# yanielc/medical-vision-textural-bias

Hardware: AMD Instinct MI355X
Metric: BraTS 4ch 240^3 vols/sec filtered+train-step @1/2/4/8 GPU; filter HBM GB/s (higher is better)
Workload: dtype f32

## Files before the change

medical-vision-textural-bias_amd/csrc/conv_gemm.hip:

```cpp
#include <hip/hip_runtime.h>

#include <cstdint>
#include <cstdlib>

#include "gemm_core.h"
#include "num_cu.h"
#include "texbias.h"

namespace {

using namespace tb::gemm;

struct CGArgs {
  const float* x;
  const float* A;
  const float* bias;
  const float* add;
  float* y;
  float* part;
  int64_t xsn, ysn, addsn;
  int64_t xbytes;
  int xsc, ysc;
  int Cin, M;
  int IDm, IH, IW;
  int OD, OH, OW;
  int YH, YW;
  int S, ymul;
  int P;
  int nsplit, kper, mtiles, ptiles, ncls;
  int kind;
  int64_t aoff[8];
  int Kc[8], Tc[8];
};

__host__ __device__ inline void tap_of(int kind, int cls, int j, int& dz, int& dy, int& dx, int& widx) {
  if (kind == 0) {
    dz = j / 9 - 1, dy = (j / 3) % 3 - 1, dx = j % 3 - 1, widx = j;
  } else if (kind == 1) {
    dz = dy = dx = 0, widx = 0;
  } else {
    const int pz = (cls >> 2) & 1, py = (cls >> 1) & 1, px = cls & 1;
    const int nx = 1 + px, ny = 1 + py;
    const int ix = j % nx, iy = (j / nx) % ny, iz = j / (nx * ny);
    dz = pz ? iz : 0, dy = py ? iy : 0, dx = px ? ix : 0;
    const int tz = pz ? (iz ? 0 : 2) : 1, ty = py ? (iy ? 0 : 2) : 1, tx = px ? (ix ? 0 : 2) : 1;
    widx = tz * 9 + ty * 3 + tx;
  }
}

template <int BM, int BP, int WGM>
__global__ __launch_bounds__(NTH) void k_conv_gemm(const CGArgs a) {
  using TileT = Tile<BM, BP, WGM>;
  constexpr int NPOS = BP / 64;
  constexpr int AQ = BM * KC / 4 / NTH;
  static_assert(NPOS >= 1 && AQ >= 1, "tile");
  extern __shared__ __attribute__((aligned(16))) float lds_dyn[];
  const int tid = (int)threadIdx.x, lane = tid & 63;
  const int w = __builtin_amdgcn_readfirstlane(tid >> 6);
  int b = xcd_remap((int)blockIdx.x, (int)gridDim.x);
  const int mt = b % a.mtiles;
  b /= a.mtiles;
  const int pt = b % a.ptiles;
  b /= a.ptiles;
  const int split = b % a.nsplit, cls = b / a.nsplit;
  const int T = a.Tc[cls], K = a.Kc[cls];
  const float* __restrict__ A = a.A + a.aoff[cls];
  const int Cin = a.Cin;
  const int k_beg = split * a.kper;
  const int k_end = min(K, k_beg + a.kper);
  const int m0 = mt * BM, p0 = pt * BP;
  const int IHW = a.IH * a.IW;

  int xo[NPOS];
  uint32_t vm[NPOS];
#pragma unroll
  for (int i = 0; i < NPOS; ++i) {
    const int p = p0 + lane + 64 * i;
    const bool ok = p < a.P;
    int t = ok ? p : 0;
    const int ox = t % a.OW;
    t /= a.OW;
    const int oy = t % a.OH;
    t /= a.OH;
    const int oz = t % a.OD, n = t / a.OD;
    const int bz = a.S * oz, by = a.S * oy, bx = a.S * ox;
    xo[i] = 4 * ((int)(n * a.xsn) + bz * IHW + by * a.IW + bx);
    uint32_t m = 0;
    for (int j = 0; j < T; ++j) {
      int dz, dy, dx, wi;
      tap_of(a.kind, cls, j, dz, dy, dx, wi);
      const int iz = bz + dz, iy = by + dy, ix = bx + dx;
      const bool v = ok && iz >= 0 && iz < a.IDm && iy >= 0 && iy < a.IH && ix >= 0 && ix < a.IW;
      m |= (v ? 1u : 0u) << j;
    }
    vm[i] = m;
  }
  const uint32_t xbytes = (uint32_t)__builtin_amdgcn_readfirstlane((int)a.xbytes);
  const __amdgpu_buffer_rsrc_t xr = __builtin_amdgcn_make_buffer_rsrc(const_cast<float*>(a.x), 0, (int)xbytes, 0x00020000);
  const int xsc4 = 4 * a.xsc;

  float rb[2][NPOS][8];
  f32x4 ra[2][AQ];
  auto gather = [&](auto SL, int k0) {
    constexpr int sl = decltype(SL)::value;
    const int k = k0 + 8 * w;
    const int t = k / Cin, c = k - t * Cin;
    const bool kin = k < k_end;
    int dz, dy, dx, wi;
    tap_of(a.kind, cls, kin ? t : 0, dz, dy, dx, wi);
    const int off = 4 * ((dz * a.IH + dy) * a.IW + dx);
    const int soff = c * xsc4;
#pragma unroll
    for (int i = 0; i < NPOS; ++i) {
      const bool v = kin && ((vm[i] >> t) & 1u);
      const int vo = v ? xo[i] + off : (int)0x80000000;
#pragma unroll
      for (int r = 0; r < 8; ++r)
        rb[sl][i][r] = __builtin_bit_cast(float, __builtin_amdgcn_raw_buffer_load_b32(xr, vo, soff + r * xsc4, 0));
    }
  };
  const uint32_t abytes = (uint32_t)__builtin_amdgcn_readfirstlane((int)(4 * (int64_t)a.M * K));
  const __amdgpu_buffer_rsrc_t ar = __builtin_amdgcn_make_buffer_rsrc(const_cast<float*>(A), 0, (int)abytes, 0x00020000);
  auto aload = [&](auto SL, int k0) {
    constexpr int sl = decltype(SL)::value;
#pragma unroll
    for (int u = 0; u < AQ; ++u) {
      const int q4 = tid + NTH * u, row = q4 % BM, kq = k0 + 4 * (q4 / BM);
      const int m = m0 + row;
      const int vo = (m < a.M && kq < k_end) ? 4 * (m * K + kq) : (int)0x80000000;
      ra[sl][u] = __builtin_bit_cast(f32x4, __builtin_amdgcn_raw_buffer_load_b128(ar, vo, 0, 0));
    }
  };
  auto load = [&](auto SL, int s) {
    gather(SL, k_beg + s * KC);
    aload(SL, k_beg + s * KC);
  };
  auto store = [&](auto SL) {
    constexpr int sl = decltype(SL)::value;
    float* L = lds_dyn + sl * TileT::LBUF;
#pragma unroll
    for (int u = 0; u < AQ; ++u) {
      const int q4 = tid + NTH * u, row = q4 % BM, c4 = q4 / BM;
      *reinterpret_cast<f32x4*>(L + row * RS + 4 * c4) = ra[sl][u];
    }
#pragma unroll
    for (int i = 0; i < NPOS; ++i) {
      float* d = L + (BM + lane + 64 * i) * RS + 8 * w;
      *reinterpret_cast<f32x4*>(d) = f32x4{rb[sl][i][0], rb[sl][i][1], rb[sl][i][2], rb[sl][i][3]};
      *reinterpret_cast<f32x4*>(d + 4) = f32x4{rb[sl][i][4], rb[sl][i][5], rb[sl][i][6], rb[sl][i][7]};
    }
  };

  TileT tile(w, lane);
  tile.run(lds_dyn, k_beg < k_end ? (k_end - k_beg + KC - 1) / KC : 0, load, store);

  const int M = a.M, P = a.P;
  if (a.nsplit > 1) {
    tile.epilogue([&](int col) {
      const int p = p0 + col;
      float* dst = a.part + ((int64_t)(cls * a.nsplit + split) * M) * P + p;
      return [=](int row, float v) {
        const int m = m0 + row;
        if (p < P && m < M) dst[(int64_t)m * P] = v;
      };
    });
    return;
  }
  const float* bias = a.bias;
  const int ysc = a.ysc;
  tile.epilogue([&](int col) {
    const int p = p0 + col;
    int t = p;
    const int ox = t % a.OW;
    t /= a.OW;
    const int oy = t % a.OH;
    t /= a.OH;
    const int oz = t % a.OD, n = t / a.OD;
    const int pc = a.kind == 2 ? cls : 0;
    const int64_t sp = ((int64_t)(a.ymul * oz + (pc >> 2)) * a.YH + (a.ymul * oy + ((pc >> 1) & 1))) * a.YW +
                       a.ymul * ox + (pc & 1);
    float* yo = a.y + n * a.ysn + sp;
    const float* ad = a.add ? a.add + n * a.addsn + sp : nullptr;
    return [=](int row, float v) {
      const int m = m0 + row;
      if (p < P && m < M) {
        v += bias ? bias[m] : 0.f;
        if (ad) v += ad[(int64_t)m * ysc];
        yo[(int64_t)m * ysc] = v;
      }
    };
  });
}

__global__ __launch_bounds__(256) void k_cg_reduce(const CGArgs a) {
  const int64_t i = (int64_t)blockIdx.x * 256 + threadIdx.x;
  const int64_t per = (int64_t)a.M * a.P;
  if (i >= per * a.ncls) return;
  const int cls = (int)(i / per);
  const int64_t r = i - cls * per;
  const int m = (int)(r / a.P), p = (int)(r - (int64_t)m * a.P);
  const float* src = a.part + (int64_t)cls * a.nsplit * per + (int64_t)m * a.P + p;
  float v = a.bias ? a.bias[m] : 0.f;
  float s = 0.f;
  for (int k = 0; k < a.nsplit; ++k) s += src[k * per];
  v += s;
  int t = p;
  const int ox = t % a.OW;
  t /= a.OW;
  const int oy = t % a.OH;
  t /= a.OH;
  const int oz = t % a.OD, n = t / a.OD;
  const int pc = a.kind == 2 ? cls : 0;
  const int64_t sp =
      ((int64_t)(a.ymul * oz + (pc >> 2)) * a.YH + (a.ymul * oy + ((pc >> 1) & 1))) * a.YW + a.ymul * ox + (pc & 1);
  if (a.add) v += a.add[n * a.addsn + (int64_t)m * a.ysc + sp];
  a.y[n * a.ysn + (int64_t)m * a.ysc + sp] = v;
}

__global__ __launch_bounds__(256) void k_cg_pack(const float* __restrict__ W, float* __restrict__ out, int mode,
                                                 int64_t total, const CGArgs a) {
  const int64_t i = (int64_t)blockIdx.x * 256 + threadIdx.x;
  if (i >= total) return;
  int cls = 0;
  while (cls + 1 < a.ncls && i >= a.aoff[cls + 1]) ++cls;
  const int64_t r = i - a.aoff[cls];
  const int Kc = a.Kc[cls], Cin = a.Cin, M = a.M;
  const int m = (int)(r / Kc), k = (int)(r - (int64_t)m * Kc);
  const int j = k / Cin, c = k - j * Cin;
  int dz, dy, dx, wi;
  tap_of(a.kind, cls, j, dz, dy, dx, wi);
  const int TW = a.kind == 1 ? 1 : 27;
  float v;
  if (mode == 0) v = W[((int64_t)m * Cin + c) * TW + wi];
  else if (mode == 1) v = W[((int64_t)c * M + m) * TW + (TW - 1 - wi)];
  else v = W[((int64_t)c * M + m) * 27 + wi];
  out[i] = v;
}

struct Plan {
  CGArgs a;
  int BM, BP, WGM;
  size_t pack_floats, part_floats;
};

inline size_t align_floats(size_t n) { return (n + 63) & ~size_t(63); }

int make_plan(int mode, int N, int Cin, int M, int D, int H, int Wd, int stride, int ksize, Plan& pl) {
  if (N < 1 || Cin < 1 || M < 1 || D < 1 || H < 1 || Wd < 1) return TB_ERR_INVALID_ARG;
  if (mode < 0 || mode > 2 || (ksize != 3 && ksize != 1) || (stride != 1 && stride != 2)) return TB_ERR_INVALID_ARG;
  if (Cin % 8 != 0) return TB_ERR_UNSUPPORTED_SIZE;
  if (mode == 2 && (ksize != 3 || stride != 2)) return TB_ERR_INVALID_ARG;
  if (mode == 1 && stride != 1) return TB_ERR_INVALID_ARG;
  CGArgs& a = pl.a;
  a = CGArgs{};
  a.Cin = Cin, a.M = M, a.IDm = D, a.IH = H, a.IW = Wd;
  a.xsc = D * H * Wd;
  if ((int64_t)N * Cin * D * H * Wd >= (int64_t)1 << 31) return TB_ERR_UNSUPPORTED_SIZE;
  if (mode == 2) {
    a.S = 1, a.ymul = 2, a.OD = D, a.OH = H, a.OW = Wd, a.YH = 2 * H, a.YW = 2 * Wd, a.ncls = 8, a.kind = 2;
    int64_t off = 0;
    for (int cls = 0; cls < 8; ++cls) {
      const int T = (1 + ((cls >> 2) & 1)) * (1 + ((cls >> 1) & 1)) * (1 + (cls & 1));
      a.Tc[cls] = T, a.Kc[cls] = Cin * T, a.aoff[cls] = off;
      off += (int64_t)M * Cin * T;
    }
    pl.pack_floats = (size_t)off;
  } else {
    const int pad = ksize == 3 ? 1 : 0;
    a.S = stride, a.ymul = 1, a.ncls = 1, a.kind = ksize == 3 ? 0 : 1;
    a.OD = (D + 2 * pad - ksize) / stride + 1, a.OH = (H + 2 * pad - ksize) / stride + 1,
    a.OW = (Wd + 2 * pad - ksize) / stride + 1;
    a.YH = a.OH, a.YW = a.OW;
    const int T = ksize * ksize * ksize;
    a.Tc[0] = T, a.Kc[0] = Cin * T, a.aoff[0] = 0;
    pl.pack_floats = (size_t)M * Cin * T;
  }
  a.ysc = a.ymul == 2 ? 8 * a.OD * a.OH * a.OW : a.OD * a.OH * a.OW;
  if ((int64_t)N * M * a.ysc >= (int64_t)1 << 31) return TB_ERR_UNSUPPORTED_SIZE;
  a.P = N * a.OD * a.OH * a.OW;
  static const int cfg[3][3] = {{32, 128, 1}, {64, 64, 2}, {128, 128, 2}};
  const int tile = M <= 32 ? 0 : (M <= 64 ? 1 : 2);
  pl.BM = cfg[tile][0], pl.BP = cfg[tile][1], pl.WGM = cfg[tile][2];
  a.mtiles = (M + pl.BM - 1) / pl.BM;
  a.ptiles = (a.P + pl.BP - 1) / pl.BP;
  int Kmax = 0;
  for (int c = 0; c < a.ncls; ++c) Kmax = a.Kc[c] > Kmax ? a.Kc[c] : Kmax;
  const int64_t base = (int64_t)a.mtiles * a.ptiles * a.ncls;
  int occ = (int)(163840 / lds_bytes(pl.BM, pl.BP));
  occ = occ > 4 ? 4 : (occ < 1 ? 1 : occ);
  const int64_t slots = (int64_t)occ * tb::num_cu();
  const int stages = (Kmax + KC - 1) / KC;
  double best = 1e30;
  int ns = 1;
  for (int s = 1; s <= 16 && s <= stages; ++s) {
    const int64_t blocks = base * s;
    const int64_t rounds = (blocks + slots - 1) / slots;
    const double cost = (double)rounds * ((stages + s - 1) / s + 3);
    if (cost < best * 0.97) best = cost, ns = s;
  }
  a.kper = ((Kmax + ns - 1) / ns + KC - 1) / KC * KC;
  a.nsplit = (Kmax + a.kper - 1) / a.kper;
  pl.part_floats = a.nsplit > 1 ? (size_t)a.ncls * a.nsplit * M * a.P : 0;
  return TB_OK;
}

template <int BM, int BP, int WGM>
hipError_t launch(const CGArgs& a, hipStream_t st) {
  const int64_t nb = (int64_t)a.mtiles * a.ptiles * a.nsplit * a.ncls;
  return launch_tile<&k_conv_gemm<BM, BP, WGM>>(lds_bytes(BM, BP), nb, a, st);
}

}

size_t tb_conv3d_gemm_workspace_bytes(int mode, int N, int Cin, int M, int D, int H, int Wd, int stride, int ksize) {
  Plan pl;
  if (make_plan(mode, N, Cin, M, D, H, Wd, stride, ksize, pl) != TB_OK) return 0;
  return 4 * (align_floats(pl.pack_floats) + align_floats(pl.part_floats)) + 256;
}

int tb_conv3d_gemm_f32(int mode, const float* x, int64_t xsn, const float* W, const float* bias, const float* add,
                       int64_t addsn, float* y, int64_t ysn, int N, int Cin, int M, int D, int H, int Wd, int stride,
                       int ksize, void* ws, size_t ws_bytes, void* stream) {
  if (!x || !W || !y) return TB_ERR_INVALID_ARG;
  Plan pl;
  const int rc = make_plan(mode, N, Cin, M, D, H, Wd, stride, ksize, pl);
  if (rc != TB_OK) return rc;
  CGArgs& a = pl.a;
  const size_t need = 4 * (align_floats(pl.pack_floats) + align_floats(pl.part_floats)) + 256;
  if (!ws || ws_bytes < need) return TB_ERR_WORKSPACE;
  hipStream_t st = reinterpret_cast<hipStream_t>(stream);
  a.x = x, a.bias = bias, a.add = add, a.y = y;
  a.xsn = xsn > 0 ? xsn : (int64_t)Cin * a.xsc;
  a.ysn = ysn > 0 ? ysn : (int64_t)M * a.ysc;
  a.addsn = addsn > 0 ? addsn : a.ysn;
  a.xbytes = 4 * ((int64_t)(N - 1) * a.xsn + (int64_t)Cin * a.xsc);
  if (a.xbytes >= (int64_t)1 << 31) return TB_ERR_UNSUPPORTED_SIZE;
  float* wsf = reinterpret_cast<float*>((reinterpret_cast<uintptr_t>(ws) + 255) & ~uintptr_t(255));
  {
    const int64_t total = (int64_t)pl.pack_floats;
    hipLaunchKernelGGL(k_cg_pack, dim3((unsigned)((total + 255) / 256)), dim3(256), 0, st, W, wsf, mode, total, a);
    a.A = wsf;
  }
  a.part = wsf + align_floats(pl.pack_floats);
  hipError_t e = hipSuccess;
  if (pl.BM == 32) e = launch<32, 128, 1>(a, st);
  else if (pl.BM == 64) e = launch<64, 64, 2>(a, st);
  else e = launch<128, 128, 2>(a, st);
  if (e != hipSuccess) return TB_ERR_HIP;
  if (a.nsplit > 1) {
    const int64_t tot = (int64_t)a.ncls * a.M * a.P;
    hipLaunchKernelGGL(k_cg_reduce, dim3((unsigned)((tot + 255) / 256)), dim3(256), 0, st, a);
    if (hipGetLastError() != hipSuccess) return TB_ERR_HIP;
  }
  return TB_OK;
}

int tb_conv3d_gemm_config(int mode, int N, int Cin, int M, int D, int H, int Wd, int stride, int ksize, int64_t* cfg) {
  Plan pl;
  const int rc = make_plan(mode, N, Cin, M, D, H, Wd, stride, ksize, pl);
  if (rc != TB_OK || !cfg) return rc != TB_OK ? rc : TB_ERR_INVALID_ARG;
  cfg[0] = pl.BM, cfg[1] = pl.BP, cfg[2] = pl.a.nsplit, cfg[3] = pl.a.kper;
  cfg[4] = (int64_t)pl.a.mtiles * pl.a.ptiles * pl.a.nsplit * pl.a.ncls;
  cfg[5] = pl.a.P;
  return TB_OK;
}
```

medical-vision-textural-bias_amd/csrc/gemm_core.h:

```cpp
#pragma once

#include <hip/hip_runtime.h>

#include <cstdint>
#include <mutex>
#include <type_traits>

namespace tb {
namespace gemm {

typedef float f32x4 __attribute__((ext_vector_type(4)));
typedef float f32x16 __attribute__((ext_vector_type(16)));

constexpr int KC = 32;
constexpr int NTH = 256;
constexpr int RS = 36;

template <int I>
using Idx = std::integral_constant<int, I>;

__device__ __forceinline__ int xcd_remap(int b, int nb) {
  const int q = nb >> 3, r = nb & 7, x = b & 7, i = b >> 3;
  return x < r ? x * (q + 1) + i : r * (q + 1) + (x - r) * q + i;
}

template <int BM, int BP, int WGM>
struct Tile {
  static constexpr int WGN = 4 / WGM;
  static constexpr int TM = BM / WGM / 32, TN = BP / WGN / 32;
  static constexpr int LBUF = (BM + BP) * RS;
  static_assert(TM >= 1 && TN >= 1, "tile");

  f32x16 acc[TM][TN];
  int wm, wn, kk, l32;

  __device__ __forceinline__ Tile(int w, int lane) : wm(w % WGM), wn(w / WGM), kk(lane >> 5), l32(lane & 31) {
#pragma unroll
    for (int tm = 0; tm < TM; ++tm)
#pragma unroll
      for (int tn = 0; tn < TN; ++tn)
#pragma unroll
        for (int r = 0; r < 16; ++r) acc[tm][tn][r] = 0.f;
  }

  template <int sl, int h>
  __device__ __forceinline__ void half(const float* lds) {
    const float* L = lds + sl * LBUF;
    f32x4 af[TM][2], bf[TN][2];
#pragma unroll
    for (int tm = 0; tm < TM; ++tm) {
      const float* src = L + ((wm * TM + tm) * 32 + l32) * RS + 16 * kk + 8 * h;
#pragma unroll
      for (int q = 0; q < 2; ++q) af[tm][q] = *reinterpret_cast<const f32x4*>(src + 4 * q);
    }
#pragma unroll
    for (int tn = 0; tn < TN; ++tn) {
      const float* src = L + (BM + (wn * TN + tn) * 32 + l32) * RS + 16 * kk + 8 * h;
#pragma unroll
      for (int q = 0; q < 2; ++q) bf[tn][q] = *reinterpret_cast<const f32x4*>(src + 4 * q);
    }
#pragma unroll
    for (int st = 0; st < 8; ++st)
#pragma unroll
      for (int tm = 0; tm < TM; ++tm)
#pragma unroll
        for (int tn = 0; tn < TN; ++tn)
          acc[tm][tn] = __builtin_amdgcn_mfma_f32_32x32x2f32(af[tm][st >> 2][st & 3], bf[tn][st >> 2][st & 3],
                                                             acc[tm][tn], 0, 0, 0);
  }

  template <class Load, class Store>
  __device__ __forceinline__ void run(const float* lds, int nst, Load&& load, Store&& store) {
    if (nst > 0) {
      load(Idx<0>{}, 0);
      store(Idx<0>{});
      load(Idx<1>{}, 1);
    }
    __syncthreads();
    for (int s = 0; s < nst; s += 2) {
      stage<0>(lds, s, load, store);
      if (s + 1 < nst) stage<1>(lds, s + 1, load, store);
    }
  }

  template <int sl, class Load, class Store>
  __device__ __forceinline__ void stage(const float* lds, int s, Load& load, Store& store) {
    half<sl, 0>(lds);
    load(Idx<sl>{}, s + 2);
    half<sl, 1>(lds);
    store(Idx<1 - sl>{});
    __syncthreads();
  }

  template <class Column>
  __device__ __forceinline__ void epilogue(Column&& column) {
#pragma unroll
    for (int tn = 0; tn < TN; ++tn) {
      auto sink = column((wn * TN + tn) * 32 + l32);
#pragma unroll
      for (int tm = 0; tm < TM; ++tm)
#pragma unroll
        for (int r = 0; r < 16; ++r) sink((wm * TM + tm) * 32 + (r & 3) + 8 * (r >> 2) + 4 * kk, acc[tm][tn][r]);
    }
  }
};

inline size_t lds_bytes(int BM, int BP) { return (size_t)2 * (BM + BP) * RS * sizeof(float); }

template <auto Kern, class Args>
hipError_t launch_tile(size_t lds, int64_t nb, const Args& a, hipStream_t st) {
  static std::once_flag once;
  static hipError_t attr = hipSuccess;
  std::call_once(once, [&] {
    attr = hipFuncSetAttribute(reinterpret_cast<const void*>(Kern), hipFuncAttributeMaxDynamicSharedMemorySize, (int)lds);
  });
  if (attr != hipSuccess) return attr;
  hipLaunchKernelGGL(Kern, dim3((unsigned)nb), dim3(NTH), lds, st, a);
  return hipGetLastError();
}

}
}
```

medical-vision-textural-bias_amd/csrc/split_bf16.h:

```cpp
#pragma once
#include <hip/hip_runtime.h>

namespace tb {

typedef __bf16 bf16x8 __attribute__((ext_vector_type(8)));
typedef __bf16 bf16x2 __attribute__((ext_vector_type(2)));
typedef float f32x2s __attribute__((ext_vector_type(2)));
typedef float f32x4s __attribute__((ext_vector_type(4)));

__device__ __forceinline__ void split3_pk(float a, float b, unsigned& p0, unsigned& p1, unsigned& p2) {
  const float top = __uint_as_float(0x7f7f7fffu);
  const bf16x2 h = __builtin_convertvector(
      f32x2s{__builtin_amdgcn_fmed3f(a, -top, top), __builtin_amdgcn_fmed3f(b, -top, top)}, bf16x2);
  p0 = __builtin_bit_cast(unsigned, h);
  const float ra = a - __uint_as_float(p0 << 16), rb = b - __uint_as_float(p0 & 0xffff0000u);
  const bf16x2 m = __builtin_convertvector(f32x2s{ra, rb}, bf16x2);
  p1 = __builtin_bit_cast(unsigned, m);
  const float sa = ra - __uint_as_float(p1 << 16), sb = rb - __uint_as_float(p1 & 0xffff0000u);
  const bf16x2 l = __builtin_convertvector(f32x2s{sa, sb}, bf16x2);
  p2 = __builtin_bit_cast(unsigned, l);
}

__device__ __forceinline__ void split3(const float (&v)[8], bf16x8& p0, bf16x8& p1, bf16x8& p2) {
  unsigned q[3][4];
#pragma unroll
  for (int j = 0; j < 4; ++j) split3_pk(v[2 * j], v[2 * j + 1], q[0][j], q[1][j], q[2][j]);
  typedef unsigned u32x4 __attribute__((ext_vector_type(4)));
  p0 = __builtin_bit_cast(bf16x8, u32x4{q[0][0], q[0][1], q[0][2], q[0][3]});
  p1 = __builtin_bit_cast(bf16x8, u32x4{q[1][0], q[1][1], q[1][2], q[1][3]});
  p2 = __builtin_bit_cast(bf16x8, u32x4{q[2][0], q[2][1], q[2][2], q[2][3]});
}

__device__ __forceinline__ void mfma_split6(const bf16x8 (&a)[3], const bf16x8 (&b)[3], f32x4s& hi, f32x4s& lo) {
  lo = __builtin_amdgcn_mfma_f32_16x16x32_bf16(a[1], b[1], lo, 0, 0, 0);
  lo = __builtin_amdgcn_mfma_f32_16x16x32_bf16(a[0], b[2], lo, 0, 0, 0);
  lo = __builtin_amdgcn_mfma_f32_16x16x32_bf16(a[2], b[0], lo, 0, 0, 0);
  lo = __builtin_amdgcn_mfma_f32_16x16x32_bf16(a[0], b[1], lo, 0, 0, 0);
  lo = __builtin_amdgcn_mfma_f32_16x16x32_bf16(a[1], b[0], lo, 0, 0, 0);
  hi = __builtin_amdgcn_mfma_f32_16x16x32_bf16(a[0], b[0], hi, 0, 0, 0);
}

}
```

Before: 180.6.

## Use split-bf16 MFMA tile with 512 threads for wide conv GEMMs

For convolutions with more than 64 output channels, the implicit-GEMM conv kernel now uses a new SplitTile. It splits f32 operands into three bf16 parts and accumulates six 32x32x16 bf16 MFMAs per k-step in hi/lo accumulators, replacing the f32 path. The weight pack kernel emits the three bf16 planes directly, and the tile runs on 512 threads with position groups. This aims to trade f32 FMA throughput for bf16 matrix-core throughput while keeping near-f32 accuracy, at the cost of more LDS traffic, register pressure and split arithmetic on the activation gather.

```diff
diff --git a/medical-vision-textural-bias_amd/csrc/conv_gemm.hip b/medical-vision-textural-bias_amd/csrc/conv_gemm.hip
--- a/medical-vision-textural-bias_amd/csrc/conv_gemm.hip
+++ b/medical-vision-textural-bias_amd/csrc/conv_gemm.hip
@@ -13,7 +13,7 @@
 
 struct CGArgs {
   const float* x;
-  const float* A;
+  const void* A;
   const float* bias;
   const float* add;
   float* y;
@@ -30,6 +30,7 @@
   int nsplit, kper, mtiles, ptiles, ncls;
   int kind;
   int64_t aoff[8];
+  int64_t apart;
   int Kc[8], Tc[8];
 };
 
@@ -48,15 +49,22 @@
   }
 }
 
-template <int BM, int BP, int WGM>
-__global__ __launch_bounds__(NTH) void k_conv_gemm(const CGArgs a) {
-  using TileT = Tile<BM, BP, WGM>;
-  constexpr int NPOS = BP / 64;
-  constexpr int AQ = BM * KC / 4 / NTH;
+template <int BM, int BP, int WGM, int NT, bool SP>
+__global__ __launch_bounds__(NT) void k_conv_gemm(const CGArgs a) {
+  using TileT = std::conditional_t<SP, SplitTile<BM, BP, WGM, NT>, Tile<BM, BP, WGM>>;
+  using LdsT = std::conditional_t<SP, char, float>;
+  typedef unsigned u32x4 __attribute__((ext_vector_type(4)));
+  static_assert(SP || NT == NTH, "the f32 tile runs on NTH threads");
+  constexpr int PG = NT / 256;
+  constexpr int NPOS = BP / (64 * PG);
+  constexpr int AQ = SP ? (BM * 4 + NT - 1) / NT
+                        : BM * KC / 4 / NT;
   static_assert(NPOS >= 1 && AQ >= 1, "tile");
-  extern __shared__ __attribute__((aligned(16))) float lds_dyn[];
+  extern __shared__ __attribute__((aligned(16))) char lds_raw[];
+  LdsT* const lds_dyn = reinterpret_cast<LdsT*>(lds_raw);
   const int tid = (int)threadIdx.x, lane = tid & 63;
   const int w = __builtin_amdgcn_readfirstlane(tid >> 6);
+  const int wk = w & 3, pg = w >> 2;
   int b = xcd_remap((int)blockIdx.x, (int)gridDim.x);
   const int mt = b % a.mtiles;
   b /= a.mtiles;
@@ -64,7 +72,6 @@
   b /= a.ptiles;
   const int split = b % a.nsplit, cls = b / a.nsplit;
   const int T = a.Tc[cls], K = a.Kc[cls];
-  const float* __restrict__ A = a.A + a.aoff[cls];
   const int Cin = a.Cin;
   const int k_beg = split * a.kper;
   const int k_end = min(K, k_beg + a.kper);
@@ -75,7 +82,7 @@
   uint32_t vm[NPOS];
 #pragma unroll
   for (int i = 0; i < NPOS; ++i) {
-    const int p = p0 + lane + 64 * i;
+    const int p = p0 + lane + 64 * (PG * i + pg);
     const bool ok = p < a.P;
     int t = ok ? p : 0;
     const int ox = t % a.OW;
@@ -100,10 +107,10 @@
   const int xsc4 = 4 * a.xsc;
 
   float rb[2][NPOS][8];
-  f32x4 ra[2][AQ];
+  std::conditional_t<SP, u32x4[2][AQ][3], f32x4[2][AQ]> ra;
   auto gather = [&](auto SL, int k0) {
     constexpr int sl = decltype(SL)::value;
-    const int k = k0 + 8 * w;
+    const int k = k0 + 8 * wk;
     const int t = k / Cin, c = k - t * Cin;
     const bool kin = k < k_end;
     int dz, dy, dx, wi;
@@ -119,16 +126,30 @@
         rb[sl][i][r] = __builtin_bit_cast(float, __builtin_amdgcn_raw_buffer_load_b32(xr, vo, soff + r * xsc4, 0));
     }
   };
-  const uint32_t abytes = (uint32_t)__builtin_amdgcn_readfirstlane((int)(4 * (int64_t)a.M * K));
-  const __amdgpu_buffer_rsrc_t ar = __builtin_amdgcn_make_buffer_rsrc(const_cast<float*>(A), 0, (int)abytes, 0x00020000);
+  const int esz = SP ? 2 : 4;
+  const char* Ab = reinterpret_cast<const char*>(a.A) + esz * a.aoff[cls];
+  const int apart2 = __builtin_amdgcn_readfirstlane((int)(2 * a.apart));
+  const uint32_t abytes =
+      (uint32_t)__builtin_amdgcn_readfirstlane((int)(esz * (int64_t)a.M * K + (SP ? 2 * (int64_t)apart2 : 0)));
+  const __amdgpu_buffer_rsrc_t ar = __builtin_amdgcn_make_buffer_rsrc(const_cast<char*>(Ab), 0, (int)abytes, 0x00020000);
   auto aload = [&](auto SL, int k0) {
     constexpr int sl = decltype(SL)::value;
 #pragma unroll
     for (int u = 0; u < AQ; ++u) {
-      const int q4 = tid + NTH * u, row = q4 % BM, kq = k0 + 4 * (q4 / BM);
-      const int m = m0 + row;
-      const int vo = (m < a.M && kq < k_end) ? 4 * (m * K + kq) : (int)0x80000000;
-      ra[sl][u] = __builtin_bit_cast(f32x4, __builtin_amdgcn_raw_buffer_load_b128(ar, vo, 0, 0));
+      if constexpr (SP) {
+        const int it = tid + NT * u, row = it % BM, kq = k0 + 8 * (it / BM);
+        const int m = m0 + row;
+        const bool v = (BM * 4 % NT == 0 || it < BM * 4) && m < a.M && kq < k_end;
+        const int vo = v ? 2 * (m * K + kq) : (int)0x80000000;
+#pragma unroll
+        for (int p = 0; p < 3; ++p)
+          ra[sl][u][p] = __builtin_bit_cast(u32x4, __builtin_amdgcn_raw_buffer_load_b128(ar, vo, p * apart2, 0));
+      } else {
+        const int q4 = tid + NT * u, row = q4 % BM, kq = k0 + 4 * (q4 / BM);
+        const int m = m0 + row;
+        const int vo = (m < a.M && kq < k_end) ? 4 * (m * K + kq) : (int)0x80000000;
+        ra[sl][u] = __builtin_bit_cast(f32x4, __builtin_amdgcn_raw_buffer_load_b128(ar, vo, 0, 0));
+      }
     }
   };
   auto load = [&](auto SL, int s) {
@@ -137,17 +158,40 @@
   };
   auto store = [&](auto SL) {
     constexpr int sl = decltype(SL)::value;
-    float* L = lds_dyn + sl * TileT::LBUF;
-#pragma unroll
-    for (int u = 0; u < AQ; ++u) {
-      const int q4 = tid + NTH * u, row = q4 % BM, c4 = q4 / BM;
-      *reinterpret_cast<f32x4*>(L + row * RS + 4 * c4) = ra[sl][u];
-    }
-#pragma unroll
-    for (int i = 0; i < NPOS; ++i) {
-      float* d = L + (BM + lane + 64 * i) * RS + 8 * w;
-      *reinterpret_cast<f32x4*>(d) = f32x4{rb[sl][i][0], rb[sl][i][1], rb[sl][i][2], rb[sl][i][3]};
-      *reinterpret_cast<f32x4*>(d + 4) = f32x4{rb[sl][i][4], rb[sl][i][5], rb[sl][i][6], rb[sl][i][7]};
+    if constexpr (SP) {
+      char* L = lds_dyn + sl * TileT::LBUF;
+#pragma unroll
+      for (int u = 0; u < AQ; ++u) {
+        const int it = tid + NT * u;
+        if (BM * 4 % NT == 0 || it < BM * 4) {
+#pragma unroll
+          for (int p = 0; p < 3; ++p)
+            *reinterpret_cast<u32x4*>(L + p * TileT::IMG + TileT::a_off(it % BM, it / BM)) = ra[sl][u][p];
+        }
+      }
+#pragma unroll
+      for (int i = 0; i < NPOS; ++i) {
+        unsigned q[3][4];
+#pragma unroll
+        for (int j = 0; j < 4; ++j) tb::split3_pk(rb[sl][i][2 * j], rb[sl][i][2 * j + 1], q[0][j], q[1][j], q[2][j]);
+        char* d = L + TileT::b_off(lane + 64 * (PG * i + pg), wk);
+#pragma unroll
+        for (int p = 0; p < 3; ++p)
+          *reinterpret_cast<u32x4*>(d + p * TileT::IMG) = u32x4{q[p][0], q[p][1], q[p][2], q[p][3]};
+      }
+    } else {
+      float* L = lds_dyn + sl * TileT::LBUF;
+#pragma unroll
+      for (int u = 0; u < AQ; ++u) {
+        const int q4 = tid + NT * u, row = q4 % BM, c4 = q4 / BM;
+        *reinterpret_cast<f32x4*>(L + row * RS + 4 * c4) = ra[sl][u];
+      }
+#pragma unroll
+      for (int i = 0; i < NPOS; ++i) {
+        float* d = L + (BM + lane + 64 * i) * RS + 8 * w;
+        *reinterpret_cast<f32x4*>(d) = f32x4{rb[sl][i][0], rb[sl][i][1], rb[sl][i][2], rb[sl][i][3]};
+        *reinterpret_cast<f32x4*>(d + 4) = f32x4{rb[sl][i][4], rb[sl][i][5], rb[sl][i][6], rb[sl][i][7]};
+      }
     }
   };
 
@@ -217,7 +261,8 @@
   a.y[n * a.ysn + (int64_t)m * a.ysc + sp] = v;
 }
 
-__global__ __launch_bounds__(256) void k_cg_pack(const float* __restrict__ W, float* __restrict__ out, int mode,
+template <bool SP>
+__global__ __launch_bounds__(256) void k_cg_pack(const float* __restrict__ W, void* __restrict__ out, int mode,
                                                  int64_t total, const CGArgs a) {
   const int64_t i = (int64_t)blockIdx.x * 256 + threadIdx.x;
   if (i >= total) return;
@@ -234,16 +279,30 @@
   if (mode == 0) v = W[((int64_t)m * Cin + c) * TW + wi];
   else if (mode == 1) v = W[((int64_t)c * M + m) * TW + (TW - 1 - wi)];
   else v = W[((int64_t)c * M + m) * 27 + wi];
-  out[i] = v;
+  if constexpr (SP) {
+    unsigned p0, p1, p2;
+    tb::split3_pk(v, 0.f, p0, p1, p2);
+    uint16_t* o = static_cast<uint16_t*>(out) + i;
+    o[0] = (uint16_t)p0, o[total] = (uint16_t)p1, o[2 * total] = (uint16_t)p2;
+  } else {
+    static_cast<float*>(out)[i] = v;
+  }
 }
 
 struct Plan {
   CGArgs a;
   int BM, BP, WGM;
+  bool split;
   size_t pack_floats, part_floats;
+  size_t pack_bytes() const { return (pack_floats * (split ? 6 : 4) + 255) & ~size_t(255); }
+  size_t ws_bytes() const { return pack_bytes() + 4 * ((part_floats + 63) & ~size_t(63)) + 256; }
 };
 
-inline size_t align_floats(size_t n) { return (n + 63) & ~size_t(63); }
+struct TileCfg {
+  int BM, BP, WGM, NT;
+  bool split;
+};
+constexpr TileCfg kTiles[3] = {{32, 128, 1, NTH, false}, {64, 64, 2, NTH, false}, {128, 128, 2, 512, true}};
 
 int make_plan(int mode, int N, int Cin, int M, int D, int H, int Wd, int stride, int ksize, Plan& pl) {
   if (N < 1 || Cin < 1 || M < 1 || D < 1 || H < 1 || Wd < 1) return TB_ERR_INVALID_ARG;
@@ -278,15 +337,16 @@
   a.ysc = a.ymul == 2 ? 8 * a.OD * a.OH * a.OW : a.OD * a.OH * a.OW;
   if ((int64_t)N * M * a.ysc >= (int64_t)1 << 31) return TB_ERR_UNSUPPORTED_SIZE;
   a.P = N * a.OD * a.OH * a.OW;
-  static const int cfg[3][3] = {{32, 128, 1}, {64, 64, 2}, {128, 128, 2}};
-  const int tile = M <= 32 ? 0 : (M <= 64 ? 1 : 2);
-  pl.BM = cfg[tile][0], pl.BP = cfg[tile][1], pl.WGM = cfg[tile][2];
+  const TileCfg& tc = kTiles[M <= 32 ? 0 : (M <= 64 ? 1 : 2)];
+  pl.BM = tc.BM, pl.BP = tc.BP, pl.WGM = tc.WGM, pl.split = tc.split;
+  a.apart = (int64_t)pl.pack_floats;
+  if (6 * (int64_t)pl.pack_floats >= (int64_t)1 << 31) return TB_ERR_UNSUPPORTED_SIZE;
   a.mtiles = (M + pl.BM - 1) / pl.BM;
   a.ptiles = (a.P + pl.BP - 1) / pl.BP;
   int Kmax = 0;
   for (int c = 0; c < a.ncls; ++c) Kmax = a.Kc[c] > Kmax ? a.Kc[c] : Kmax;
   const int64_t base = (int64_t)a.mtiles * a.ptiles * a.ncls;
-  int occ = (int)(163840 / lds_bytes(pl.BM, pl.BP));
+  int occ = (int)(163840 / (pl.split ? split_lds_bytes(pl.BM, pl.BP) : lds_bytes(pl.BM, pl.BP)));
   occ = occ > 4 ? 4 : (occ < 1 ? 1 : occ);
   const int64_t slots = (int64_t)occ * tb::num_cu();
   const int stages = (Kmax + KC - 1) / KC;
@@ -304,10 +364,12 @@
   return TB_OK;
 }
 
-template <int BM, int BP, int WGM>
+template <int I>
 hipError_t launch(const CGArgs& a, hipStream_t st) {
+  constexpr TileCfg c = kTiles[I];
   const int64_t nb = (int64_t)a.mtiles * a.ptiles * a.nsplit * a.ncls;
-  return launch_tile<&k_conv_gemm<BM, BP, WGM>>(lds_bytes(BM, BP), nb, a, st);
+  return launch_tile<&k_conv_gemm<c.BM, c.BP, c.WGM, c.NT, c.split>, c.NT>(
+      c.split ? split_lds_bytes(c.BM, c.BP) : lds_bytes(c.BM, c.BP), nb, a, st);
 }
 
 }
@@ -315,7 +377,7 @@
 size_t tb_conv3d_gemm_workspace_bytes(int mode, int N, int Cin, int M, int D, int H, int Wd, int stride, int ksize) {
   Plan pl;
   if (make_plan(mode, N, Cin, M, D, H, Wd, stride, ksize, pl) != TB_OK) return 0;
-  return 4 * (align_floats(pl.pack_floats) + align_floats(pl.part_floats)) + 256;
+  return pl.ws_bytes();
 }
 
 int tb_conv3d_gemm_f32(int mode, const float* x, int64_t xsn, const float* W, const float* bias, const float* add,
@@ -326,8 +388,7 @@
   const int rc = make_plan(mode, N, Cin, M, D, H, Wd, stride, ksize, pl);
   if (rc != TB_OK) return rc;
   CGArgs& a = pl.a;
-  const size_t need = 4 * (align_floats(pl.pack_floats) + align_floats(pl.part_floats)) + 256;
-  if (!ws || ws_bytes < need) return TB_ERR_WORKSPACE;
+  if (!ws || ws_bytes < pl.ws_bytes()) return TB_ERR_WORKSPACE;
   hipStream_t st = reinterpret_cast<hipStream_t>(stream);
   a.x = x, a.bias = bias, a.add = add, a.y = y;
   a.xsn = xsn > 0 ? xsn : (int64_t)Cin * a.xsc;
@@ -335,17 +396,19 @@
   a.addsn = addsn > 0 ? addsn : a.ysn;
   a.xbytes = 4 * ((int64_t)(N - 1) * a.xsn + (int64_t)Cin * a.xsc);
   if (a.xbytes >= (int64_t)1 << 31) return TB_ERR_UNSUPPORTED_SIZE;
-  float* wsf = reinterpret_cast<float*>((reinterpret_cast<uintptr_t>(ws) + 255) & ~uintptr_t(255));
+  char* wsb = reinterpret_cast<char*>((reinterpret_cast<uintptr_t>(ws) + 255) & ~uintptr_t(255));
   {
     const int64_t total = (int64_t)pl.pack_floats;
-    hipLaunchKernelGGL(k_cg_pack, dim3((unsigned)((total + 255) / 256)), dim3(256), 0, st, W, wsf, mode, total, a);
-    a.A = wsf;
-  }
-  a.part = wsf + align_floats(pl.pack_floats);
+    const dim3 grid((unsigned)((total + 255) / 256));
+    if (pl.split) hipLaunchKernelGGL(k_cg_pack<true>, grid, dim3(256), 0, st, W, (void*)wsb, mode, total, a);
+    else hipLaunchKernelGGL(k_cg_pack<false>, grid, dim3(256), 0, st, W, (void*)wsb, mode, total, a);
+    a.A = wsb;
+  }
+  a.part = reinterpret_cast<float*>(wsb + pl.pack_bytes());
   hipError_t e = hipSuccess;
-  if (pl.BM == 32) e = launch<32, 128, 1>(a, st);
-  else if (pl.BM == 64) e = launch<64, 64, 2>(a, st);
-  else e = launch<128, 128, 2>(a, st);
+  if (pl.BM == 32) e = launch<0>(a, st);
+  else if (pl.BM == 64) e = launch<1>(a, st);
+  else e = launch<2>(a, st);
   if (e != hipSuccess) return TB_ERR_HIP;
   if (a.nsplit > 1) {
     const int64_t tot = (int64_t)a.ncls * a.M * a.P;
diff --git a/medical-vision-textural-bias_amd/csrc/gemm_core.h b/medical-vision-textural-bias_amd/csrc/gemm_core.h
--- a/medical-vision-textural-bias_amd/csrc/gemm_core.h
+++ b/medical-vision-textural-bias_amd/csrc/gemm_core.h
@@ -5,6 +5,8 @@
 #include <cstdint>
 #include <mutex>
 #include <type_traits>
+
+#include "split_bf16.h"
 
 namespace tb {
 namespace gemm {
@@ -107,7 +109,91 @@
 
 inline size_t lds_bytes(int BM, int BP) { return (size_t)2 * (BM + BP) * RS * sizeof(float); }
 
-template <auto Kern, class Args>
+constexpr int SRS = 80;
+
+template <int BM, int BP, int WGM, int NT>
+struct SplitTile {
+  static constexpr int NW = NT / 64, WGN = NW / WGM;
+  static constexpr int TM = BM / WGM / 32, TN = BP / WGN / 32;
+  static constexpr int IMG = (BM + BP) * SRS;
+  static constexpr int LBUF = 3 * IMG;
+  static_assert(TM >= 1 && TN >= 1 && WGM * WGN * 64 == NT, "tile");
+
+  f32x16s hi[TM][TN], lo[TM][TN];
+  int wm, wn, kk, l32;
+
+  __device__ __forceinline__ SplitTile(int w, int lane) : wm(w % WGM), wn(w / WGM), kk(lane >> 5), l32(lane & 31) {
+#pragma unroll
+    for (int tm = 0; tm < TM; ++tm)
+#pragma unroll
+      for (int tn = 0; tn < TN; ++tn)
+#pragma unroll
+        for (int r = 0; r < 16; ++r) hi[tm][tn][r] = 0.f, lo[tm][tn][r] = 0.f;
+  }
+
+  static __device__ __forceinline__ int a_off(int row, int oct) { return row * SRS + 16 * oct; }
+  static __device__ __forceinline__ int b_off(int row, int oct) { return (BM + row) * SRS + 16 * oct; }
+
+  template <int sl, int ks>
+  __device__ __forceinline__ void half(const char* lds) {
+    const char* L = lds + sl * LBUF + 32 * ks + 16 * kk;
+    bf16x8 af[TM][3], bf[TN][3];
+#pragma unroll
+    for (int tm = 0; tm < TM; ++tm)
+#pragma unroll
+      for (int p = 0; p < 3; ++p)
+        af[tm][p] = *reinterpret_cast<const bf16x8*>(L + p * IMG + ((wm * TM + tm) * 32 + l32) * SRS);
+#pragma unroll
+    for (int tn = 0; tn < TN; ++tn)
+#pragma unroll
+      for (int p = 0; p < 3; ++p)
+        bf[tn][p] = *reinterpret_cast<const bf16x8*>(L + p * IMG + (BM + (wn * TN + tn) * 32 + l32) * SRS);
+#pragma unroll
+    for (int tm = 0; tm < TM; ++tm)
+#pragma unroll
+      for (int tn = 0; tn < TN; ++tn) mfma_split6_32(af[tm], bf[tn], hi[tm][tn], lo[tm][tn]);
+  }
+
+  template <class Load, class Store>
+  __device__ __forceinline__ void run(const char* lds, int nst, Load&& load, Store&& store) {
+    if (nst > 0) {
+      load(Idx<0>{}, 0);
+      store(Idx<0>{});
+      load(Idx<1>{}, 1);
+    }
+    __syncthreads();
+    for (int s = 0; s < nst; s += 2) {
+      stage<0>(lds, s, load, store);
+      if (s + 1 < nst) stage<1>(lds, s + 1, load, store);
+    }
+  }
+
+  template <int sl, class Load, class Store>
+  __device__ __forceinline__ void stage(const char* lds, int s, Load& load, Store& store) {
+    half<sl, 0>(lds);
+    load(Idx<sl>{}, s + 2);
+    half<sl, 1>(lds);
+    store(Idx<1 - sl>{});
+    __syncthreads();
+  }
+
+  template <class Column>
+  __device__ __forceinline__ void epilogue(Column&& column) {
+#pragma unroll
+    for (int tn = 0; tn < TN; ++tn) {
+      auto sink = column((wn * TN + tn) * 32 + l32);
+#pragma unroll
+      for (int tm = 0; tm < TM; ++tm)
+#pragma unroll
+        for (int r = 0; r < 16; ++r)
+          sink((wm * TM + tm) * 32 + (r & 3) + 8 * (r >> 2) + 4 * kk, hi[tm][tn][r] + lo[tm][tn][r]);
+    }
+  }
+};
+
+inline size_t split_lds_bytes(int BM, int BP) { return (size_t)2 * 3 * (BM + BP) * SRS; }
+
+template <auto Kern, int NT = NTH, class Args>
 hipError_t launch_tile(size_t lds, int64_t nb, const Args& a, hipStream_t st) {
   static std::once_flag once;
   static hipError_t attr = hipSuccess;
@@ -115,7 +201,7 @@
     attr = hipFuncSetAttribute(reinterpret_cast<const void*>(Kern), hipFuncAttributeMaxDynamicSharedMemorySize, (int)lds);
   });
   if (attr != hipSuccess) return attr;
-  hipLaunchKernelGGL(Kern, dim3((unsigned)nb), dim3(NTH), lds, st, a);
+  hipLaunchKernelGGL(Kern, dim3((unsigned)nb), dim3(NT), lds, st, a);
   return hipGetLastError();
 }
 
diff --git a/medical-vision-textural-bias_amd/csrc/split_bf16.h b/medical-vision-textural-bias_amd/csrc/split_bf16.h
--- a/medical-vision-textural-bias_amd/csrc/split_bf16.h
+++ b/medical-vision-textural-bias_amd/csrc/split_bf16.h
@@ -40,4 +40,15 @@
   hi = __builtin_amdgcn_mfma_f32_16x16x32_bf16(a[0], b[0], hi, 0, 0, 0);
 }
 
+typedef float f32x16s __attribute__((ext_vector_type(16)));
+
+__device__ __forceinline__ void mfma_split6_32(const bf16x8 (&a)[3], const bf16x8 (&b)[3], f32x16s& hi, f32x16s& lo) {
+  lo = __builtin_amdgcn_mfma_f32_32x32x16_bf16(a[1], b[1], lo, 0, 0, 0);
+  lo = __builtin_amdgcn_mfma_f32_32x32x16_bf16(a[0], b[2], lo, 0, 0, 0);
+  lo = __builtin_amdgcn_mfma_f32_32x32x16_bf16(a[2], b[0], lo, 0, 0, 0);
+  lo = __builtin_amdgcn_mfma_f32_32x32x16_bf16(a[0], b[1], lo, 0, 0, 0);
+  lo = __builtin_amdgcn_mfma_f32_32x32x16_bf16(a[1], b[0], lo, 0, 0, 0);
+  hi = __builtin_amdgcn_mfma_f32_32x32x16_bf16(a[0], b[0], hi, 0, 0, 0);
 }
+
+}
```

Result: faster. 183.7 (median of 6 runs) (+1.7%).
